# WeiZhang1988/YDORBSLAM

Measured on AMD Instinct MI355X. Metric: ORB extract+match Mkeypoints/sec, higher is better.
Workload: dtype u8

## Files before the change

ydorbslam_amd/csrc/extract_kernels.hip.h:

```cpp
#pragma once
#include <hip/hip_runtime.h>
#include <stdint.h>

#include "quadtree_core.h"
#include "quadtree_flat.h"

#pragma clang fp contract(off)

namespace ydorb {

constexpr int kPad = 19;
constexpr int kBorder = 16;
constexpr int kMaxLevels = 8;
constexpr int kTileMax = 72;
#ifndef QT_THREADS
#define QT_THREADS 512
#endif
constexpr int kQtThreads = QT_THREADS;

struct LevelDev {
  int w, h, pitch;
  int padOff;
  int blurOff, blurPitch;
  int cellBegin, nCells;
  int quota;
  int candOff;
  int kpOff;
  int tabOff;
  int nodeTabOff;
  float scale;
  float size;
};
struct PlanDev {
  int nLevels, nCellsTotal, cellCap, sumQuota;
  int maxX[16];
  unsigned nodeTabFrameStride;
  int blurTileBegin[kMaxLevels + 1];
  int borderBegin[kMaxLevels + 1];
  LevelDev lv[kMaxLevels];
};
#ifndef BLUR_TH
#define BLUR_TH 58
#endif
constexpr int kBlurTW = 64, kBlurTH = BLUR_TH;
struct CellDev {
  short level, x0, y0, x1, y1, pad0;
  int srcOff;
};

__device__ __forceinline__ int reflect101(int i, int n) {
  if (n == 1) return 0;
  while (i < 0 || i >= n) i = i < 0 ? -i : 2 * (n - 1) - i;
  return i;
}

typedef uint32_t __attribute__((aligned(1))) u32_unaligned;
typedef unsigned long long __attribute__((aligned(1))) u64_unaligned;

#ifndef PYR_ROWS
#define PYR_ROWS 8
#endif
constexpr int kPyrRows = PYR_ROWS;
__global__ __launch_bounds__(256) void k_pyr_level0(const uint8_t* __restrict__ img, int stride, size_t frameStride,
                                                    uint8_t* __restrict__ pyr, size_t pyrFrameStride, LevelDev L) {
  const int wx = blockIdx.x * 64 + (threadIdx.x & 63);
  const int yb = (blockIdx.y * 4 + __builtin_amdgcn_readfirstlane(threadIdx.x >> 6)) * kPyrRows;
  const int x0 = wx * 4 - kPad;
  if (x0 + 3 < 0 || x0 >= L.w) return;
  const uint8_t* src = img + (size_t)blockIdx.z * frameStride;
  uint8_t* dst = pyr + (size_t)blockIdx.z * pyrFrameStride + L.padOff + (size_t)kPad * L.pitch + wx * 4;
  const int xa = L.w >= 4 ? min(max(x0, 0), L.w - 4) : 0, sh = 8 * (x0 - xa);
  uint32_t v[kPyrRows];
#pragma unroll
  for (int r = 0; r < kPyrRows; r++) {
    const uint8_t* row = src + (size_t)min(yb + r, L.h - 1) * stride;
    if (L.w >= 4) {
      v[r] = *reinterpret_cast<const u32_unaligned*>(row + xa);
    } else {
      v[r] = 0;
      for (int b = 0; b < L.w; b++) v[r] |= (uint32_t)row[b] << (8 * b);
    }
    v[r] = sh < 0 ? v[r] << (-sh) : v[r] >> sh;
  }
#pragma unroll
  for (int r = 0; r < kPyrRows; r++)
    if (yb + r < L.h) *reinterpret_cast<uint32_t*>(dst + (size_t)(yb + r) * L.pitch) = v[r];
}

__global__ __launch_bounds__(256) void k_pyr_resize(uint8_t* __restrict__ pyr, size_t pyrFrameStride, LevelDev Lp, LevelDev L,
                                                    double scaleX, const short* __restrict__ alpha,
                                                    const int* __restrict__ yofs, const short* __restrict__ beta) {
  const int wx = blockIdx.x * 64 + (threadIdx.x & 63);
  const int yb = (blockIdx.y * 4 + __builtin_amdgcn_readfirstlane(threadIdx.x >> 6)) * kPyrRows;
  const int x0 = wx * 4 - kPad;
  if (x0 + 3 < 0 || x0 >= L.w) return;
  uint8_t* frame = pyr + (size_t)blockIdx.z * pyrFrameStride;
  const uint8_t* S = frame + Lp.padOff + (size_t)kPad * Lp.pitch + kPad;
  uint8_t* dst = frame + L.padOff + (size_t)kPad * L.pitch + wx * 4;
  int sx[4], sx1[4], a0[4], a1[4];
#pragma unroll
  for (int b = 0; b < 4; b++) {
    const int dx = min(max(x0 + b, 0), L.w - 1);
    const float fx = (float)__dsub_rn(__dmul_rn((double)dx + 0.5, scaleX), 0.5);
    sx[b] = min(max((int)floorf(fx), 0), Lp.w - 1);
    a0[b] = alpha[2 * dx]; a1[b] = alpha[2 * dx + 1];
    sx1[b] = min(sx[b] + 1, Lp.w - 1);
  }
  const bool fast = sx[3] - sx[0] <= 6;
  const uint8_t *r0p[kPyrRows], *r1p[kPyrRows];
  int b0[kPyrRows], b1[kPyrRows];
#pragma unroll
  for (int r = 0; r < kPyrRows; r++) {
    const int dy = min(yb + r, L.h - 1);
    const int sy = yofs[dy];
    b0[r] = beta[2 * dy]; b1[r] = beta[2 * dy + 1];
    r0p[r] = S + (size_t)min(max(sy, 0), Lp.h - 1) * Lp.pitch;
    r1p[r] = S + (size_t)min(max(sy + 1, 0), Lp.h - 1) * Lp.pitch;
  }
  uint32_t v[kPyrRows];
  if (fast) {
    typedef unsigned short u16x2 __attribute__((ext_vector_type(2)));
    uint32_t sel[4];
    u16x2 ab[4];
#pragma unroll
    for (int b = 0; b < 4; b++) {
      const uint32_t off = (uint32_t)(sx[b] - sx[0]);
      sel[b] = off | 0x0c000c00u | ((off + 1) << 16);
      ab[b] = u16x2{(unsigned short)a0[b], (unsigned short)a1[b]};
    }
    unsigned long long w0[kPyrRows], w1[kPyrRows];
#pragma unroll
    for (int r = 0; r < kPyrRows; r++) {
      w0[r] = *reinterpret_cast<const u64_unaligned*>(r0p[r] + sx[0]);
      w1[r] = *reinterpret_cast<const u64_unaligned*>(r1p[r] + sx[0]);
    }
#pragma unroll
    for (int r = 0; r < kPyrRows; r++) {
      v[r] = 0;
#pragma unroll
      for (int b = 0; b < 4; b++) {
        const uint32_t p0 = __builtin_amdgcn_perm((uint32_t)(w0[r] >> 32), (uint32_t)w0[r], sel[b]);
        const uint32_t p1 = __builtin_amdgcn_perm((uint32_t)(w1[r] >> 32), (uint32_t)w1[r], sel[b]);
        const int h0 = (int)__builtin_amdgcn_udot2(__builtin_bit_cast(u16x2, p0), ab[b], 0u, false);
        const int h1 = (int)__builtin_amdgcn_udot2(__builtin_bit_cast(u16x2, p1), ab[b], 0u, false);
        const int o = (((b0[r] * (h0 >> 4)) >> 16) + ((b1[r] * (h1 >> 4)) >> 16) + 2) >> 2;
        v[r] |= (uint32_t)(o & 0xFF) << (8 * b);
      }
    }
  } else {
#pragma unroll
    for (int r = 0; r < kPyrRows; r++) {
      v[r] = 0;
#pragma unroll
      for (int b = 0; b < 4; b++) {
        const int h0 = r0p[r][sx[b]] * a0[b] + r0p[r][sx1[b]] * a1[b];
        const int h1 = r1p[r][sx[b]] * a0[b] + r1p[r][sx1[b]] * a1[b];
        const int o = (((b0[r] * (h0 >> 4)) >> 16) + ((b1[r] * (h1 >> 4)) >> 16) + 2) >> 2;
        v[r] |= (uint32_t)(o & 0xFF) << (8 * b);
      }
    }
  }
#pragma unroll
  for (int r = 0; r < kPyrRows; r++)
    if (yb + r < L.h) *reinterpret_cast<uint32_t*>(dst + (size_t)(yb + r) * L.pitch) = v[r];
}

struct PyrPadEntry { uint32_t laneA4, laneB4, selM, selF; };
struct PyrColEntry { uint32_t sel[4]; uint32_t ab[4]; };
constexpr uint32_t kPermIdentity = 0x03020100u;
#ifndef PYR_ROWS_F
#define PYR_ROWS_F 8
#endif
constexpr int kPyrRowsF = PYR_ROWS_F;

__device__ __forceinline__ uint32_t pyr_finish_dword(uint32_t v, const PyrPadEntry& pe) {
  const uint32_t A = (uint32_t)__builtin_amdgcn_ds_bpermute((int)pe.laneA4, (int)v);
  const uint32_t B = (uint32_t)__builtin_amdgcn_ds_bpermute((int)pe.laneB4, (int)v);
  const uint32_t M = __builtin_amdgcn_perm(A, B, pe.selM);
  return __builtin_amdgcn_perm(M, v, pe.selF);
}
__device__ __forceinline__ void pyr_store_rows(uint8_t* dst, int pitch, int y, int h, uint32_t v) {
  if (y >= h) return;
  *reinterpret_cast<uint32_t*>(dst + (ptrdiff_t)y * pitch) = v;
  if (y >= 1 && y <= kPad) *reinterpret_cast<uint32_t*>(dst - (ptrdiff_t)y * pitch) = v;
  if (y >= h - 1 - kPad && y <= h - 2) *reinterpret_cast<uint32_t*>(dst + (ptrdiff_t)(2 * (h - 1) - y) * pitch) = v;
}

__global__ __launch_bounds__(256) void k_pyr_level0_f(const uint8_t* __restrict__ img, int stride, size_t frameStride,
                                                      uint8_t* __restrict__ pyr, size_t pyrFrameStride, LevelDev L,
                                                      const PyrPadEntry* __restrict__ padTab, int shift) {
  const int wx = blockIdx.x * 64 + (threadIdx.x & 63) - shift;
  const int yb = (blockIdx.y * 4 + __builtin_amdgcn_readfirstlane(threadIdx.x >> 6)) * kPyrRowsF;
  const int nd = (L.w + 2 * kPad + 3) >> 2;
  if (wx < 0 || wx >= nd) return;
  const int x0 = wx * 4 - kPad;
  const uint8_t* src = img + (size_t)blockIdx.z * frameStride;
  uint8_t* dst = pyr + (size_t)blockIdx.z * pyrFrameStride + L.padOff + (size_t)kPad * L.pitch + wx * 4;
  typedef uint32_t u32x4 __attribute__((ext_vector_type(4)));
  const u32x4 peRaw = reinterpret_cast<const u32x4*>(padTab)[wx];
  const PyrPadEntry pe{peRaw.x, peRaw.y, peRaw.z, peRaw.w};
  const int xa = min(max(x0, 0), L.w - 4), sh = 8 * (x0 - xa);
  uint32_t v[kPyrRowsF];
#pragma unroll
  for (int r = 0; r < kPyrRowsF; r++) {
    const uint8_t* row = src + (size_t)min(yb + r, L.h - 1) * stride;
    v[r] = *reinterpret_cast<const u32_unaligned*>(row + xa);
  }
  const int shl = min(max(-sh, 0), 31), shr = min(max(sh, 0), 31);
#pragma unroll
  for (int r = 0; r < kPyrRowsF; r++) v[r] = sh < 0 ? v[r] << shl : v[r] >> shr;
  if (__builtin_amdgcn_ballot_w64(pe.selF != kPermIdentity)) {
#pragma unroll
    for (int r = 0; r < kPyrRowsF; r++) v[r] = pyr_finish_dword(v[r], pe);
  }
#pragma unroll
  for (int r = 0; r < kPyrRowsF; r++) pyr_store_rows(dst, L.pitch, yb + r, L.h, v[r]);
}

__global__ __launch_bounds__(256) void k_pyr_resize_f(uint8_t* __restrict__ pyr, size_t pyrFrameStride, LevelDev Lp, LevelDev L,
                                                      double scaleX, const PyrColEntry* __restrict__ colTab,
                                                      const PyrPadEntry* __restrict__ padTab, const int2* __restrict__ rowTab, int shift) {
  const int wx = blockIdx.x * 64 + (threadIdx.x & 63) - shift;
  const int yb = (blockIdx.y * 4 + __builtin_amdgcn_readfirstlane(threadIdx.x >> 6)) * kPyrRowsF;
  const int nd = (L.w + 2 * kPad + 3) >> 2;
  if (wx < 0 || wx >= nd) return;
  uint8_t* frame = pyr + (size_t)blockIdx.z * pyrFrameStride;
  const uint8_t* S = frame + Lp.padOff + (size_t)kPad * Lp.pitch + kPad;
  uint8_t* dst = frame + L.padOff + (size_t)kPad * L.pitch + wx * 4;
  const int dx0 = min(max(wx * 4 - kPad, 0), L.w - 1);
  const float fx = (float)__dsub_rn(__dmul_rn((double)dx0 + 0.5, scaleX), 0.5);
  const int base = min(max((int)floorf(fx), 0), Lp.w - 1);
  const uint8_t* Sb = S + base;
  unsigned long long w0[kPyrRowsF], w1[kPyrRowsF];
  int bw[kPyrRowsF];
#pragma unroll
  for (int r = 0; r < kPyrRowsF; r++) {
    const int2 rt = rowTab[yb + r];
    bw[r] = rt.y;
    w0[r] = *reinterpret_cast<const u64_unaligned*>(Sb + (size_t)min(max(rt.x, 0), Lp.h - 1) * Lp.pitch);
    w1[r] = *reinterpret_cast<const u64_unaligned*>(Sb + (size_t)min(max(rt.x + 1, 0), Lp.h - 1) * Lp.pitch);
  }
  const PyrColEntry ce = colTab[wx];
  typedef uint32_t u32x4 __attribute__((ext_vector_type(4)));
  const u32x4 peRaw = reinterpret_cast<const u32x4*>(padTab)[wx];
  const PyrPadEntry pe{peRaw.x, peRaw.y, peRaw.z, peRaw.w};
  typedef unsigned short u16x2 __attribute__((ext_vector_type(2)));
  uint32_t v[kPyrRowsF];
#pragma unroll
  for (int r = 0; r < kPyrRowsF; r++) {
    const int b0 = bw[r] & 0xffff, b1 = (int)((uint32_t)bw[r] >> 16);
    v[r] = 0;
#pragma unroll
    for (int b = 0; b < 4; b++) {
      const uint32_t p0 = __builtin_amdgcn_perm((uint32_t)(w0[r] >> 32), (uint32_t)w0[r], ce.sel[b]);
      const uint32_t p1 = __builtin_amdgcn_perm((uint32_t)(w1[r] >> 32), (uint32_t)w1[r], ce.sel[b]);
      const int h0 = (int)__builtin_amdgcn_udot2(__builtin_bit_cast(u16x2, p0), __builtin_bit_cast(u16x2, ce.ab[b]), 0u, false);
      const int h1 = (int)__builtin_amdgcn_udot2(__builtin_bit_cast(u16x2, p1), __builtin_bit_cast(u16x2, ce.ab[b]), 0u, false);
      const int o = (((b0 * (h0 >> 4)) >> 16) + ((b1 * (h1 >> 4)) >> 16) + 2) >> 2;
      v[r] |= (uint32_t)(o & 0xFF) << (8 * b);
    }
  }
  if (__builtin_amdgcn_ballot_w64(pe.selF != kPermIdentity)) {
#pragma unroll
    for (int r = 0; r < kPyrRowsF; r++) v[r] = pyr_finish_dword(v[r], pe);
  }
#pragma unroll
  for (int r = 0; r < kPyrRowsF; r++) pyr_store_rows(dst, L.pitch, yb + r, L.h, v[r]);
}

__global__ __launch_bounds__(256) void k_pyr_borders(uint8_t* __restrict__ pyr, size_t pyrFrameStride, PlanDev P) {
  const int f = blockIdx.y;
  int t = blockIdx.x * 256 + threadIdx.x, level = 0;
#pragma unroll
  for (int l = 1; l < kMaxLevels; l++)
    if (l < P.nLevels && (int)(blockIdx.x * 256) >= P.borderBegin[l]) level = l;
  t -= P.borderBegin[level];
  const LevelDev L = P.lv[level];
  const int wd = L.pitch >> 2, rightStart = (kPad + L.w) >> 2;
  constexpr int xdLo = (kPad + 3) / 4;
  const int xdEnd = min(rightStart, wd);
  const int nFast = max(xdEnd - xdLo, 0), nEdge = wd - nFast;
  uint8_t* base = pyr + (size_t)f * pyrFrameStride + L.padOff;
  if (t < 2 * kPad * nFast) {
    const int r = t / nFast, xf = xdLo + t - r * nFast;
    const int yy = r < kPad ? r : L.h + r;
    const int rr = reflect101(yy - kPad, L.h);
    reinterpret_cast<uint32_t*>(base + (size_t)yy * L.pitch)[xf] = reinterpret_cast<const uint32_t*>(base + (size_t)(rr + kPad) * L.pitch)[xf];
    return;
  }
  t -= 2 * kPad * nFast;
  int y, xd;
  if (t < 2 * kPad * nEdge) {
    const int r = t / nEdge, k = t - r * nEdge;
    xd = nFast == 0 ? k : (k < xdLo ? k : xdEnd + k - xdLo);
    y = r < kPad ? r : L.h + r;
  } else {
    const int u = t - 2 * kPad * nEdge, row = u / 12, j = u - row * 12;
    if (row >= L.h) return;
    y = kPad + row;
    xd = j < 6 ? j : rightStart + j - 6;
    if (xd >= wd || (j < 6 && (4 * xd >= kPad || xd >= rightStart))) return;
  }
  uint32_t* dw = reinterpret_cast<uint32_t*>(base + (size_t)y * L.pitch) + xd;
  const int Y = y - kPad, ry = reflect101(Y, L.h);
  const bool rowInside = Y >= 0 && Y < L.h;
  const uint32_t old = rowInside ? *dw : 0u;
  const uint8_t* srow = base + (size_t)(ry + kPad) * L.pitch + kPad;
  uint32_t v = 0;
#pragma unroll
  for (int b = 0; b < 4; b++) {
    const int X = 4 * xd + b - kPad;
    uint32_t px = 0;
    if (X < L.w + kPad) px = (rowInside && X >= 0 && X < L.w) ? (old >> (8 * b)) & 255u : srow[reflect101(X, L.w)];
    v |= px << (8 * b);
  }
  *dw = v;
}

typedef short s16x2 __attribute__((ext_vector_type(2)));
__device__ __forceinline__ s16x2 pk_swap(s16x2 x) { return __builtin_shufflevector(x, x, 1, 0); }
__device__ __forceinline__ s16x2 pk_min(s16x2 a, s16x2 b) { return __builtin_elementwise_min(a, b); }
__device__ __forceinline__ s16x2 pk_max(s16x2 a, s16x2 b) { return __builtin_elementwise_max(a, b); }
__device__ __forceinline__ int fast_arc_best(const s16x2 (&P)[8]) {
  s16x2 pre[8], suf[8];
  pre[0] = P[0];
#pragma unroll
  for (int j = 1; j < 8; j++) pre[j] = pk_min(pre[j - 1], P[j]);
  suf[7] = P[7];
#pragma unroll
  for (int j = 6; j >= 0; j--) suf[j] = pk_min(suf[j + 1], P[j]);
  s16x2 m[8];
#pragma unroll
  for (int j = 0; j < 8; j++) m[j] = pk_min(suf[j], pk_swap(pre[j]));
  const s16x2 r = pk_max(pk_max(pk_max(m[0], m[1]), pk_max(m[2], m[3])), pk_max(pk_max(m[4], m[5]), pk_max(m[6], m[7])));
  return max((int)r.x, (int)r.y);
}

__device__ __forceinline__ int wave_rank(unsigned long long m) {
  return (int)__builtin_amdgcn_mbcnt_hi((unsigned)(m >> 32), __builtin_amdgcn_mbcnt_lo((unsigned)m, 0u));
}

struct FastLds { int tileBytes, scoreBytes, listBytes; };

template <int PITCH>
__global__ __launch_bounds__(256) void k_fast_cells(const uint8_t* __restrict__ pyr, size_t pyrFrameStride, PlanDev P,
                                                    const CellDev* __restrict__ cells, int cellFirst, int cellEnd, int thr, FastLds lds,
                                                    uint32_t* __restrict__ cellCount, uint32_t* __restrict__ cellCand) {
// ... 494 lines not shown
    const uint2 q = *reinterpret_cast<const QT_LDS uint2*>(hist + qf_off(d + 1) + 4 * b);
    const unsigned c0 = q.x & 0xFFFFu, c1 = q.x >> 16, c2 = q.y & 0xFFFFu, c3 = q.y >> 16;
    const unsigned sum = c0 + c1 + c2 + c3;
    hist[qf_off(d) + b] = (uint16_t)sum;
    if (sum >= 2) {
      const unsigned long long nn = (c0 != 0) + (c1 != 0) + (c2 != 0) + (c3 != 0), ll = (c0 == 1) + (c1 == 1) + (c2 == 1) + (c3 == 1);
      const int dd = d + 1;
      if (dd <= 4) { tn0 += nn << (16 * (dd - 1)); tl0 += ll << (16 * (dd - 1)); }
      else { tn1 += nn << (16 * (dd - 5)); tl1 += ll << (16 * (dd - 5)); }
    }
  };
#pragma unroll
  for (int q = 0; q < 4; q++) reduce_level(5, tid + NT * q);
  __syncthreads();
  reduce_level(4, tid);
  __syncthreads();
  if (wv == 0) {
    reduce_level(3, lane);
    __builtin_amdgcn_fence(__ATOMIC_ACQ_REL, "workgroup"); __builtin_amdgcn_wave_barrier();
    if (lane < 16) reduce_level(2, lane);
    __builtin_amdgcn_fence(__ATOMIC_ACQ_REL, "workgroup"); __builtin_amdgcn_wave_barrier();
    if (lane < 4) reduce_level(1, lane);
    __builtin_amdgcn_fence(__ATOMIC_ACQ_REL, "workgroup"); __builtin_amdgcn_wave_barrier();
    if (lane == 0) reduce_level(0, 0);
  }
  tn0 = wave_sum_u64(tn0); tn1 = wave_sum_u64(tn1); tl0 = wave_sum_u64(tl0); tl1 = wave_sum_u64(tl1);
  if (lane == 0) {
    __hip_atomic_fetch_add(&sRed[0], tn0, __ATOMIC_RELAXED, __HIP_MEMORY_SCOPE_WORKGROUP);
    __hip_atomic_fetch_add(&sRed[1], tn1, __ATOMIC_RELAXED, __HIP_MEMORY_SCOPE_WORKGROUP);
    __hip_atomic_fetch_add(&sRed[2], tl0, __ATOMIC_RELAXED, __HIP_MEMORY_SCOPE_WORKGROUP);
    __hip_atomic_fetch_add(&sRed[3], tl1, __ATOMIC_RELAXED, __HIP_MEMORY_SCOPE_WORKGROUP);
  }
  __syncthreads();
  int Pn, K = 0;
  {
    int nodes[D + 1], leaves[D + 1];
    nodes[0] = 1; leaves[0] = 0;
    const unsigned long long a0 = sRed[0], a1 = sRed[1], b0 = sRed[2], b1 = sRed[3];
#pragma unroll
    for (int d = 1; d <= D; d++) {
      nodes[d] = (int)(((d <= 4 ? a0 : a1) >> (16 * ((d - 1) & 3))) & 0xFFFF);
      leaves[d] = (int)(((d <= 4 ? b0 : b1) >> (16 * ((d - 1) & 3))) & 0xFFFF);
    }
    Pn = qt_flat_passes(nodes, leaves, quota, &K, D);
  }
  const bool pairs = Pn < 1;
  if (pairs && n > kQfSmall) { give_up(); return; }
  int nOut = K < quota ? K : quota;
  if (pairs) {
    constexpr int DP = kQtPairDepth, PER = kQfSmall / NT;
    QT_LDS uint32_t* key30 = (QT_LDS uint32_t*)smem;
    QT_LDS unsigned long long* R64 = (QT_LDS unsigned long long*)(smem + 4 * kQfSmall);
    QT_LDS uint8_t* firstOf = (QT_LDS uint8_t*)(smem + 12 * kQfSmall);
    __shared__ int sDiff[kQtPairDepth + 3], sLeaf[kQtPairDepth + 2];
    const int n4 = (n + 3) & ~3;
    uint32_t kk[PER];
    __syncthreads();
    if (tid < DP + 3) sDiff[tid] = 0;
    if (tid < DP + 2) sLeaf[tid] = 0;
#pragma unroll
    for (int t = 0; t < PER; t++) {
      const int i = t * NT + tid;
      kk[t] = i < n ? qt_path_key<kQtPairDepth>(fetch(i), rootX1, rootY1) : 0xFFFFFFFFu;
      if (i < n4) key30[i] = kk[t];
    }
    __syncthreads();
    int sA[PER], eA[PER];
#pragma unroll
    for (int t = 0; t < PER; t++) { sA[t] = 0; eA[t] = 0; }
    for (int q = 0; q < n4; q += 4) {
      const uint4 kq = *reinterpret_cast<const QT_LDS uint4*>(key30 + q);
      const uint32_t ko[4] = {kq.x, kq.y, kq.z, kq.w};
#pragma unroll
      for (int u = 0; u < 4; u++)
#pragma unroll
        for (int t = 0; t < PER; t++) {
          const int i = t * NT + tid;
          const uint32_t x = kk[t] ^ ko[u];
          const int dpt = q + u == i ? 0 : (x ? ((__clz((int)x) - 2) >> 1) + 1 : DP + 1);
          sA[t] = max(sA[t], dpt);
          if (q + u < i) eA[t] = max(eA[t], dpt);
        }
    }
#pragma unroll
    for (int t = 0; t < PER; t++)
      if (t * NT + tid < n) {
        if (eA[t] <= DP) { atomicAdd(&sDiff[eA[t]], 1); atomicAdd(&sDiff[min(sA[t], DP) + 1], -1); }
        if (sA[t] <= DP) atomicAdd(&sLeaf[sA[t]], 1);
      }
    __syncthreads();
    {
      int nodes[DP + 1], leaves[DP + 1], run2 = 0;
#pragma unroll
      for (int d = 0; d <= DP; d++) { run2 += sDiff[d]; nodes[d] = run2; leaves[d] = sLeaf[d]; }
      Pn = qt_flat_passes(nodes, leaves, quota, &K, DP);
    }
    if (Pn < 1) { give_up(); return; }
    nOut = K < quota ? K : quota;
    unsigned long long RR[PER];
#pragma unroll
    for (int t = 0; t < PER; t++) {
      const int i = t * NT + tid, dA = min(Pn, sA[t]);
      RR[t] = ((unsigned long long)(Pn - dA) << (2 * Pn)) | (unsigned long long)((kk[t] >> (2 * (DP - dA))) ^ qt_flat_mask(dA));
      if (i < n4) R64[i] = i < n ? RR[t] : ~0ull;
    }
    __syncthreads();
    bool fst[PER];
#pragma unroll
    for (int t = 0; t < PER; t++) fst[t] = true;
    for (int q = 0; q < n4; q += 2) {
      const ulonglong2 o = *reinterpret_cast<const QT_LDS ulonglong2*>(R64 + q);
      const unsigned long long oo[2] = {o.x, o.y};
#pragma unroll
      for (int u = 0; u < 2; u++)
#pragma unroll
        for (int t = 0; t < PER; t++) fst[t] = fst[t] && !(oo[u] == RR[t] && q + u < t * NT + tid);
    }
#pragma unroll
    for (int t = 0; t < PER; t++) { const int i = t * NT + tid; if (i < n4) firstOf[i] = i < n && fst[t]; }
    __syncthreads();
    int kp[PER], mm[PER];
#pragma unroll
    for (int t = 0; t < PER; t++) { kp[t] = 0; mm[t] = 0; }
    for (int q = 0; q < n4; q += 2) {
      const ulonglong2 o = *reinterpret_cast<const QT_LDS ulonglong2*>(R64 + q);
      const unsigned long long oo[2] = {o.x, o.y};
      const unsigned f2 = *reinterpret_cast<const QT_LDS uint16_t*>(firstOf + q);
#pragma unroll
      for (int u = 0; u < 2; u++)
#pragma unroll
        for (int t = 0; t < PER; t++) {
          kp[t] += (oo[u] < RR[t]) & ((f2 >> (8 * u)) & 1u);
          mm[t] += oo[u] == RR[t];
        }
    }
#pragma unroll
    for (int t = 0; t < PER; t++) {
      const int i = t * NT + tid;
      if (i < n && kp[t] < nOut && mm[t] > 16) nodeBig[kp[t]] = 1;
    }
    static_assert(PER <= ITEMS, "the all-pairs candidates live in the first PER state registers");
#pragma unroll
    for (int t = 0; t < PER; t++) st[t] = (st[t] & 0xFFFF0000u) | (uint32_t)(kp[t] < nOut ? kp[t] : 0x7FFF);
    __syncthreads();
  }

#pragma unroll
  for (int g = 0; g < ITEMS / 4; g++) {
    if (!pairs && 4 * g * NT < n) {
      int key[4], slot[4];
#pragma unroll
      for (int jj = 0; jj < 4; jj++) { key[jj] = (int)(st[4 * g + jj] & 0xFFFu); slot[jj] = qf_off(Pn) + (key[jj] >> (2 * (D - Pn))); }
      for (int d = Pn - 1; d >= 1; d--) {
        const int off = qf_off(d), sh = 2 * (D - d);
#pragma unroll
        for (int jj = 0; jj < 4; jj++) {
          const int sl = off + (key[jj] >> sh);
          if (hist[sl] == 1) slot[jj] = sl;
        }
      }
#pragma unroll
      for (int jj = 0; jj < 4; jj++) st[4 * g + jj] = (st[4 * g + jj] & 0xFFFF0000u) | (uint32_t)slot[jj];
    }
  }
  if (!pairs) {
    const int TQ = ((1 << (2 * Pn)) - 1) / 3;
    const int per = (TQ + NT - 1) / NT;
    constexpr int MAXQ = ((1 << (2 * D)) - 1) / 3 / NT + 1;
    uint2 qv[MAXQ];
    int qslot[MAXQ];
    unsigned flags = 0, cntF = 0;
#pragma unroll
    for (int t = 0; t < MAXQ; t++) {
      qslot[t] = -1; qv[t] = make_uint2(0, 0);
      const int q = tid * per + t;
      if (t < per && q < TQ) {
        int d = Pn, start = 0;
        while (q >= start + (1 << (2 * (d - 1)))) { start += 1 << (2 * (d - 1)); d--; }
        const int pq = q - start;
        const int bq = pq ^ (int)(qt_flat_mask(d) >> 2);
        qslot[t] = qf_off(d) + 4 * bq;
        qv[t] = *reinterpret_cast<const QT_LDS uint2*>(hist + qslot[t]);
        const unsigned c[4] = {qv[t].x & 0xFFFFu, qv[t].x >> 16, qv[t].y & 0xFFFFu, qv[t].y >> 16};
        const unsigned sum = c[0] + c[1] + c[2] + c[3];
#pragma unroll
        for (int e = 0; e < 4; e++) {
          const unsigned cn = c[3 - e];
          const bool fl = sum >= 2 && (d == Pn ? cn >= 1 : cn == 1);
          flags |= (unsigned)fl << (4 * t + e);
          cntF += fl;
        }
      }
    }
    unsigned total;
    unsigned pos = block_scan_excl(cntF, &total);
    if ((int)total != K) { give_up(); return; }
#pragma unroll
    for (int t = 0; t < MAXQ; t++) {
      if (qslot[t] >= 0) {
        const unsigned c[4] = {qv[t].x & 0xFFFFu, qv[t].x >> 16, qv[t].y & 0xFFFFu, qv[t].y >> 16};
        unsigned o[4];
#pragma unroll
        for (int e = 0; e < 4; e++) {
          const unsigned cn = c[3 - e];
          unsigned v = 0x7FFFu;
          if ((flags >> (4 * t + e)) & 1u) {
            if ((int)pos < nOut) {
              v = pos | (cn > 16 ? 0x8000u : 0u);
              if (cn > 16) nodeBig[pos] = 1;
            }
            pos++;
          }
          o[3 - e] = v;
        }
        *reinterpret_cast<QT_LDS uint2*>(hist + qslot[t]) = make_uint2(o[0] | (o[1] << 16), o[2] | (o[3] << 16));
      }
    }
  }
  __syncthreads();

#pragma unroll
  for (int g = 0; g < ITEMS / 4; g++) {
    if (4 * g * NT < n) {
      unsigned pv[4];
#pragma unroll
      for (int jj = 0; jj < 4; jj++) pv[jj] = pairs ? st[4 * g + jj] & 0x7FFFu : hist[st[4 * g + jj] & 0xFFFFu] & 0x7FFFu;
#pragma unroll
      for (int jj = 0; jj < 4; jj++) {
        const int i = (4 * g + jj) * NT + tid;
        const bool ok = i < n && (int)pv[jj] < nOut;
        const unsigned k = ok ? pv[jj] : (unsigned)(quotaMax + 1);
        const uint32_t rs = st[4 * g + jj] & 0xFFFF0000u;
        __hip_atomic_fetch_max(nodeLo + k, ok ? rs | (0xFFFFu - (uint32_t)i) : 0u, __ATOMIC_RELAXED, __HIP_MEMORY_SCOPE_WORKGROUP);
        __hip_atomic_fetch_max(nodeHi + k, ok ? rs | (uint32_t)i : 0u, __ATOMIC_RELAXED, __HIP_MEMORY_SCOPE_WORKGROUP);
        st[4 * g + jj] = rs | (ok ? k : 0xFFFFu);
      }
    }
  }
  __syncthreads();
  for (int k = tid; k < nOut; k += NT) {
    const unsigned iLo = 0xFFFFu - (nodeLo[k] & 0xFFFFu), iHi = nodeHi[k] & 0xFFFFu;
    if (iLo == iHi || !nodeBig[k]) {
      outKp[k] = fetch((int)iLo);
    } else {
      const int s = atomicAdd(&sTieN, 1);
      if (s < kQfMaxTied) { sTieNode[s] = k; nodeBig[k] = (uint8_t)(2 + s); }
    }
  }
  __syncthreads();
  const int nTied = sTieN;
  if (nTied > kQfMaxTied) { give_up(); return; }
  if (nTied > 0) {
    const int slotCap = kQfTieCap / nTied;
    QT_LDS uint32_t* tKey = (QT_LDS uint32_t*)smem;
    QT_LDS uint32_t* tVal = tKey + kQfTieCap;
#pragma unroll
    for (int j = 0; j < ITEMS; j++) {
      if (j * NT < n) {
        const unsigned k = st[j] & 0xFFFFu;
        if (k != 0xFFFFu) {
          const unsigned tb = nodeBig[k];
          if (tb >= 2) {
            const int s = (int)tb - 2, idx = atomicAdd(&sTieCnt[s], 1);
            if (idx < slotCap) { tKey[s * slotCap + idx] = (uint32_t)(j * NT + tid); tVal[s * slotCap + idx] = st[j] >> 16; }
            else sFlag = 1;
          }
        }
      }
    }
    __syncthreads();
    if (sFlag) { give_up(); return; }
    for (int s = 0; s < nTied; s++) {
      const int m = sTieCnt[s];
      constexpr int MAXM = (kQfTieCap + NT - 1) / NT;
      int rk[MAXM];
      uint32_t oi[MAXM], rr[MAXM];
#pragma unroll
      for (int t = 0; t < MAXM; t++) {
        rk[t] = -1; oi[t] = 0; rr[t] = 0;
        const int e = tid + NT * t;
        if (e < m) {
          oi[t] = tKey[s * slotCap + e];
          rr[t] = tVal[s * slotCap + e];
          int r = 0;
          for (int u = 0; u < m; u++) r += tKey[s * slotCap + u] < oi[t];
          rk[t] = r;
        }
      }
      __syncthreads();
#pragma unroll
      for (int t = 0; t < MAXM; t++)
        if (rk[t] >= 0) { tKey[s * slotCap + rk[t]] = (rr[t] << 16) | (uint32_t)rk[t]; tVal[s * slotCap + rk[t]] = oi[t]; }
      __syncthreads();
    }
    if (tid < nTied) {
      const int m = sTieCnt[tid];
      const int best = qt_sort_front(tKey + tid * slotCap, m);
      outKp[sTieNode[tid]] = fetch((int)tVal[tid * slotCap + best]);
    }
  }
  if (tid == 0) { needPass[unit] = 0; lvlCount[unit] = nOut; }
}

__global__ __launch_bounds__(256) void k_blur(const uint8_t* __restrict__ pyr, size_t pyrFrameStride, uint8_t* __restrict__ blur,
                                              size_t blurFrameStride, PlanDev P) {
  constexpr int TW = kBlurTW, TH = kBlurTH, SH = TH + 6, SWW = 18;
  __shared__ uint32_t src[SH * SWW];
  __shared__ __align__(16) uint32_t hb[(SH / 2) * TW];
  int f = blockIdx.y, tileId = blockIdx.x;
  if ((f | 7) < (int)gridDim.y) {
    tileId = (f & 7) * (gridDim.x >> 3) + (blockIdx.x >> 3);
    f = (f & ~7) | (blockIdx.x & 7);
  }
  if (tileId >= P.blurTileBegin[P.nLevels]) return;
  int level = 0;
#pragma unroll
  for (int l = 1; l < kMaxLevels; l++)
    if (l < P.nLevels && tileId >= P.blurTileBegin[l]) level = l;
  tileId -= P.blurTileBegin[level];
  const LevelDev L = P.lv[level];
  const int tilesX = (L.w + TW - 1) / TW;
  const int ty = tileId / tilesX, tx = tileId - ty * tilesX;
  const int x0 = tx * TW, y0 = ty * TH;
  const uint8_t* padded = pyr + (size_t)f * pyrFrameStride + L.padOff;
  {
    const int r0 = threadIdx.x / SWW, wd = threadIdx.x - r0 * SWW;
    const int pcol = x0 + 16 + 4 * wd;
    const bool colOk = pcol < L.pitch;
    if (r0 < 14)
#pragma unroll
      for (int r = r0; r < SH; r += 14) {
        const int prow = min(y0 + r + kPad - 3, L.h + 2 * kPad - 1);
        src[r * SWW + wd] = colOk ? *reinterpret_cast<const uint32_t*>(padded + (size_t)prow * L.pitch + pcol) : 0u;
      }
  }
  __syncthreads();
  for (int task = threadIdx.x; task < (SH / 2) * (TW / 4); task += 256) {
    const int rp = task >> 4, g = task & 15;
    uint32_t o[2][4];
#pragma unroll
    for (int h = 0; h < 2; h++) {
      const int r = 2 * rp + h;
      const uint32_t w0 = src[r * SWW + g], w1 = src[r * SWW + g + 1], w2 = src[r * SWW + g + 2];
#pragma unroll
      for (int k = 0; k < 4; k++) {
        const uint32_t lo4 = k ? __builtin_amdgcn_alignbyte(w1, w0, k) : w0, hi4 = k ? __builtin_amdgcn_alignbyte(w2, w1, k) : w1;
        o[h][k] = __builtin_amdgcn_udot4(hi4, 0x00122230u, __builtin_amdgcn_udot4(lo4, 0x38302212u, 0u, false), false);
      }
    }
    *reinterpret_cast<uint4*>(&hb[rp * TW + g * 4]) =
        make_uint4(o[0][0] | (o[1][0] << 16), o[0][1] | (o[1][1] << 16), o[0][2] | (o[1][2] << 16), o[0][3] | (o[1][3] << 16));
  }
  __syncthreads();
  const int c4 = (threadIdx.x & 15) * 4;
#pragma unroll
  for (int r = threadIdx.x >> 4; r < TH; r += 16) {
    const int gy = y0 + r;
    if (!(gy < L.h && x0 + c4 < L.blurPitch)) continue;
    typedef unsigned short u16x2 __attribute__((ext_vector_type(2)));
    const bool odd = r & 1;
    const u16x2 k0 = odd ? u16x2{0, 18} : u16x2{18, 34}, k1 = odd ? u16x2{34, 48} : u16x2{48, 56};
    const u16x2 k2 = odd ? u16x2{56, 48} : u16x2{48, 34}, k3 = odd ? u16x2{34, 18} : u16x2{18, 0};
    const uint32_t* hp = &hb[(r >> 1) * TW + c4];
    const uint4 p0 = *reinterpret_cast<const uint4*>(hp), p1 = *reinterpret_cast<const uint4*>(hp + TW);
    const uint4 p2 = *reinterpret_cast<const uint4*>(hp + 2 * TW), p3 = *reinterpret_cast<const uint4*>(hp + 3 * TW);
    const uint32_t q0[4] = {p0.x, p0.y, p0.z, p0.w}, q1[4] = {p1.x, p1.y, p1.z, p1.w}, q2[4] = {p2.x, p2.y, p2.z, p2.w}, q3[4] = {p3.x, p3.y, p3.z, p3.w};
    uint32_t acc[4];
#pragma unroll
    for (int k = 0; k < 4; k++) {
      acc[k] = __builtin_amdgcn_udot2(__builtin_bit_cast(u16x2, q0[k]), k0, 32768u, false);
      acc[k] = __builtin_amdgcn_udot2(__builtin_bit_cast(u16x2, q1[k]), k1, acc[k], false);
      acc[k] = __builtin_amdgcn_udot2(__builtin_bit_cast(u16x2, q2[k]), k2, acc[k], false);
      acc[k] = __builtin_amdgcn_udot2(__builtin_bit_cast(u16x2, q3[k]), k3, acc[k], false);
    }
    const uint32_t out = (acc[0] >> 16) | ((acc[1] >> 16) << 8) | ((acc[2] >> 16) << 16) | ((acc[3] >> 16) << 24);
    *reinterpret_cast<uint32_t*>(blur + (size_t)f * blurFrameStride + L.blurOff + (size_t)gy * L.blurPitch + x0 + c4) = out;
  }
}

__device__ __forceinline__ float fast_atan2_deg(float y, float x) {
  const float p1 = 0.9997878412794807f * (float)(180 / 3.14159265358979323846);
  const float p3 = -0.3258083974640975f * (float)(180 / 3.14159265358979323846);
  const float p5 = 0.1555786518463281f * (float)(180 / 3.14159265358979323846);
  const float p7 = -0.04432655554792128f * (float)(180 / 3.14159265358979323846);
  const float eps = (float)2.2204460492503131e-16;
  const float ax = fabsf(x), ay = fabsf(y);
  float a, c, c2;
  if (ax >= ay) {
    c = __fdiv_rn(ay, __fadd_rn(ax, eps));
    c2 = __fmul_rn(c, c);
    a = __fmul_rn(__fadd_rn(__fmul_rn(__fadd_rn(__fmul_rn(__fadd_rn(__fmul_rn(p7, c2), p5), c2), p3), c2), p1), c);
  } else {
    c = __fdiv_rn(ax, __fadd_rn(ay, eps));
    c2 = __fmul_rn(c, c);
    a = __fsub_rn(90.f, __fmul_rn(__fadd_rn(__fmul_rn(__fadd_rn(__fmul_rn(__fadd_rn(__fmul_rn(p7, c2), p5), c2), p3), c2), p1), c));
  }
  if (x < 0) a = __fsub_rn(180.f, a);
  if (y < 0) a = __fsub_rn(360.f, a);
  return a;
}

__device__ __forceinline__ void sincos_det(float xf, float* sinOut, float* cosOut) {
  const double x = (double)xf;
  const double n = rint(__dmul_rn(x, 6.36619772367581382433e-01));
  const double r = __dsub_rn(__dsub_rn(x, __dmul_rn(n, 1.57079632673412561417e+00)), __dmul_rn(n, 6.07710050650619224932e-11));
  const double z = __dmul_rn(r, r);
  double p = __dmul_rn(z, 1.58969099521155010221e-10);
  p = __dadd_rn(p, -2.50507602534068634195e-08); p = __dmul_rn(p, z);
  p = __dadd_rn(p, 2.75573137070700676789e-06);  p = __dmul_rn(p, z);
  p = __dadd_rn(p, -1.98412698298579493134e-04); p = __dmul_rn(p, z);
  p = __dadd_rn(p, 8.33333333332248946124e-03);  p = __dmul_rn(p, z);
  p = __dadd_rn(p, -1.66666666666666324348e-01); p = __dmul_rn(p, z);
  p = __dmul_rn(p, r); p = __dadd_rn(p, r);
  double q = __dmul_rn(z, -1.13596475577881948265e-11);
  q = __dadd_rn(q, 2.08757232129817482790e-09);  q = __dmul_rn(q, z);
  q = __dadd_rn(q, -2.75573143513906633035e-07); q = __dmul_rn(q, z);
  q = __dadd_rn(q, 2.48015872894767294178e-05);  q = __dmul_rn(q, z);
  q = __dadd_rn(q, -1.38888888888741095749e-03); q = __dmul_rn(q, z);
  q = __dadd_rn(q, 4.16666666666666019037e-02);  q = __dmul_rn(q, z);
  q = __dmul_rn(q, z);
  double h = __dmul_rn(z, 0.5);
  h = __dsub_rn(h, q);
  h = __dsub_rn(1.0, h);
  const int quad = ((int)n) & 3;
  const double sv = quad == 0 ? p : quad == 1 ? h : quad == 2 ? -p : -h;
  const double cv = quad == 0 ? h : quad == 1 ? -p : quad == 2 ? -h : p;
  *sinOut = (float)sv;
  *cosOut = (float)cv;
}

__device__ __align__(16) const float kPatternDev[1024] = {
#include "orb_pattern_data.inc"
};

struct YdKeyPointDev { float x, y, size, angle, response; int octave, class_id; };

__global__ __launch_bounds__(256) void k_orient_describe(const uint8_t* __restrict__ pyr, size_t pyrFrameStride,
                                                         const uint8_t* __restrict__ blur, size_t blurFrameStride, PlanDev P,
                                                         const uint32_t* __restrict__ lvlKp, const int* __restrict__ lvlCount,
                                                         YdKeyPointDev* __restrict__ kps, uint8_t* __restrict__ desc, int cap,
                                                         int* __restrict__ nOut, float* __restrict__ lvlAngle) {
  const int lane = threadIdx.x & 63;
  int bx = blockIdx.x, f = blockIdx.y;
  if ((f | 7) < (int)gridDim.y) {
    bx = (f & 7) * (gridDim.x >> 3) + (blockIdx.x >> 3);
    f = (f & ~7) | (blockIdx.x & 7);
  }
  const int slot = bx * 4 + __builtin_amdgcn_readfirstlane(threadIdx.x >> 6);
  if (slot >= P.sumQuota) return;
  float4 pat[4];
#pragma unroll
  for (int t = 0; t < 4; t++) pat[t] = reinterpret_cast<const float4*>(kPatternDev)[t * 64 + lane];
  int level = 0;
#pragma unroll
  for (int l = 1; l < kMaxLevels; l++)
    if (l < P.nLevels && slot >= P.lv[l].kpOff) level = l;
  const uint32_t pk = __builtin_amdgcn_readfirstlane(lvlKp[(size_t)f * P.sumQuota + slot]);
  int before = 0, tot = 0, mine = 0;
#pragma unroll
  for (int l = 0; l < kMaxLevels; l++) {
    const int c = l < P.nLevels ? lvlCount[f * kMaxLevels + l] : 0;
    if (l < level) before += c;
    if (l == level) mine = c;
    tot += c;
  }
  if (slot == 0 && lane == 0) nOut[f] = min(tot, cap);
  const LevelDev L = P.lv[level];
  const int k = slot - L.kpOff;
  if (k >= mine) return;
  const int outIdx = before + k;
  if (outIdx >= cap) return;
  const int kx = qt_x(pk) + kBorder, ky = qt_y(pk) + kBorder;
  const uint8_t* roi = pyr + (size_t)f * pyrFrameStride + L.padOff + (size_t)kPad * L.pitch + kPad;
  const uint8_t* org = roi + (ptrdiff_t)(ky - 15) * L.pitch + (kx - 32);
  const int u = lane - 32;
  unsigned narrow = 0;
#pragma unroll
  for (int v = 1; v <= 15; v++) narrow |= (unsigned)(P.maxX[v] == 0) << v;
  int m10 = 0, m01 = 0;
  if (u >= -15 && u <= 15) m10 = u * org[(unsigned)(15 * L.pitch + lane)];
  if (lane >= 1 && lane <= 15 && ((narrow >> lane) & 1u)) {
    const int pos = org[(unsigned)((15 + lane) * L.pitch + 32)], neg = org[(unsigned)((15 - lane) * L.pitch + 32)];
    m01 = lane * (pos - neg);
  }
#pragma unroll
  for (int v = 1; v <= 15; v++) {
    const int d = P.maxX[v];
    if (d > 0 && u >= -d && u <= d) {
      const int pos = org[(unsigned)((15 + v) * L.pitch + lane)], neg = org[(unsigned)((15 - v) * L.pitch + lane)];
      m01 += v * (pos - neg);
      m10 += u * (pos + neg);
    }
  }
#pragma unroll
  for (int o = 32; o >= 1; o >>= 1) {
    m10 += __shfl_xor(m10, o, 64);
    m01 += __shfl_xor(m01, o, 64);
  }
  const float angle = fast_atan2_deg((float)m01, (float)m10);
  const float rad = __fmul_rn(angle, (float)(3.14159265358979323846 / 180.0));
  float sinB, cosA;
  sincos_det(rad, &sinB, &cosA);
  constexpr int kBias = 24;
  const uint8_t* bl = blur + (size_t)f * blurFrameStride + L.blurOff + (ptrdiff_t)(ky - kBias) * L.blurPitch + (kx - kBias);
  unsigned long long words[4];
#pragma unroll
  for (int t = 0; t < 4; t++) {
    const float4 pt = pat[t];
    const int r0 = __float2int_rn(__fadd_rn(__fmul_rn(pt.x, sinB), __fmul_rn(pt.y, cosA)));
    const int c0 = __float2int_rn(__fsub_rn(__fmul_rn(pt.x, cosA), __fmul_rn(pt.y, sinB)));
    const int r1 = __float2int_rn(__fadd_rn(__fmul_rn(pt.z, sinB), __fmul_rn(pt.w, cosA)));
    const int c1 = __float2int_rn(__fsub_rn(__fmul_rn(pt.z, cosA), __fmul_rn(pt.w, sinB)));
    const int t0 = bl[(unsigned)((r0 + kBias) * L.blurPitch + c0 + kBias)], t1 = bl[(unsigned)((r1 + kBias) * L.blurPitch + c1 + kBias)];
    words[t] = __ballot(t0 < t1);
  }
  if (lane < 4) {
    unsigned long long w = lane == 0 ? words[0] : lane == 1 ? words[1] : lane == 2 ? words[2] : words[3];
    reinterpret_cast<unsigned long long*>(desc + ((size_t)f * cap + outIdx) * 32)[lane] = w;
  }
  if (lane == 0) {
    YdKeyPointDev kp;
    kp.x = (float)kx;
    kp.y = (float)ky;
    if (level) { kp.x = __fmul_rn(kp.x, L.scale); kp.y = __fmul_rn(kp.y, L.scale); }
    kp.size = L.size;
    kp.angle = angle;
    kp.response = (float)qt_r(pk);
    kp.octave = level;
    kp.class_id = -1;
    kps[(size_t)f * cap + outIdx] = kp;
    lvlAngle[(size_t)f * P.sumQuota + slot] = angle;
  }
}


template <int KPW>
__global__ __launch_bounds__(256) void k_orient_describe_n(const uint8_t* __restrict__ pyr, size_t pyrFrameStride,
                                                           const uint8_t* __restrict__ blur, size_t blurFrameStride, PlanDev P,
                                                           const uint32_t* __restrict__ lvlKp, const int* __restrict__ lvlCount,
                                                           YdKeyPointDev* __restrict__ kps, uint8_t* __restrict__ desc, int cap,
                                                           int* __restrict__ nOut, float* __restrict__ lvlAngle) {
  const int lane = threadIdx.x & 63;
  int bx = blockIdx.x, f = blockIdx.y;
  if ((f | 7) < (int)gridDim.y) {
    bx = (f & 7) * (gridDim.x >> 3) + (blockIdx.x >> 3);
    f = (f & ~7) | (blockIdx.x & 7);
  }
  const int slot0 = (bx * 4 + __builtin_amdgcn_readfirstlane(threadIdx.x >> 6)) * KPW;
  if (slot0 >= P.sumQuota) return;
  float4 pat[4];
#pragma unroll
  for (int t = 0; t < 4; t++) pat[t] = reinterpret_cast<const float4*>(kPatternDev)[t * 64 + lane];
  int cnt[kMaxLevels], tot = 0;
#pragma unroll
  for (int l = 0; l < kMaxLevels; l++) { cnt[l] = l < P.nLevels ? lvlCount[f * kMaxLevels + l] : 0; tot += cnt[l]; }
  int level[KPW], outIdx[KPW];
  uint32_t pk[KPW];
  bool valid[KPW];
#pragma unroll
  for (int j = 0; j < KPW; j++) {
    const int slot = min(slot0 + j, P.sumQuota - 1);
    level[j] = 0;
#pragma unroll
    for (int l = 1; l < kMaxLevels; l++)
      if (l < P.nLevels && slot >= P.lv[l].kpOff) level[j] = l;
    pk[j] = __builtin_amdgcn_readfirstlane(lvlKp[(size_t)f * P.sumQuota + slot]);
  }
  if (slot0 == 0 && lane == 0) nOut[f] = min(tot, cap);
  bool any = false;
#pragma unroll
  for (int j = 0; j < KPW; j++) {
    int before = 0, mine = 0;
#pragma unroll
    for (int l = 0; l < kMaxLevels; l++) {
      if (l < level[j]) before += cnt[l];
      if (l == level[j]) mine = cnt[l];
    }
    const int k = slot0 + j - P.lv[level[j]].kpOff;
    outIdx[j] = before + k;
    valid[j] = slot0 + j < P.sumQuota && k < mine && outIdx[j] < cap;
    any = any || valid[j];
  }
  if (!any) return;
  int firstValid = 0;
#pragma unroll
  for (int j = KPW - 1; j >= 0; j--) if (valid[j]) firstValid = j;
#pragma unroll
  for (int j = 0; j < KPW; j++)
    if (!valid[j]) {
#pragma unroll
      for (int i = 0; i < KPW; i++) if (i == firstValid) { pk[j] = pk[i]; level[j] = level[i]; }
    }
  int kx[KPW], ky[KPW], pitch[KPW];
  const uint8_t* org[KPW];
#pragma unroll
  for (int j = 0; j < KPW; j++) {
    const LevelDev& L = P.lv[level[j]];
    kx[j] = qt_x(pk[j]) + kBorder; ky[j] = qt_y(pk[j]) + kBorder;
    pitch[j] = L.pitch;
    const uint8_t* roi = pyr + (size_t)f * pyrFrameStride + L.padOff + (size_t)kPad * L.pitch + kPad;
    org[j] = roi + (ptrdiff_t)(ky[j] - 15) * L.pitch + (kx[j] - 32);
  }
  const int u = lane - 32;
  unsigned narrow = 0;
#pragma unroll
  for (int v = 1; v <= 15; v++) narrow |= (unsigned)(P.maxX[v] == 0) << v;
  int m10[KPW], m01[KPW];
#pragma unroll
  for (int j = 0; j < KPW; j++) {
    m10[j] = 0; m01[j] = 0;
    if (u >= -15 && u <= 15) m10[j] = u * org[j][(unsigned)(15 * pitch[j] + lane)];
    if (lane >= 1 && lane <= 15 && ((narrow >> lane) & 1u)) {
      const int pos = org[j][(unsigned)((15 + lane) * pitch[j] + 32)], neg = org[j][(unsigned)((15 - lane) * pitch[j] + 32)];
      m01[j] = lane * (pos - neg);
    }
  }
#pragma unroll
  for (int v = 1; v <= 15; v++) {
    const int d = P.maxX[v];
    if (d > 0 && u >= -d && u <= d) {
#pragma unroll
      for (int j = 0; j < KPW; j++) {
        const int pos = org[j][(unsigned)((15 + v) * pitch[j] + lane)], neg = org[j][(unsigned)((15 - v) * pitch[j] + lane)];
        m01[j] += v * (pos - neg);
        m10[j] += u * (pos + neg);
      }
    }
  }
#pragma unroll
  for (int o = 32; o >= 1; o >>= 1) {
#pragma unroll
    for (int j = 0; j < KPW; j++) {
      m10[j] += __shfl_xor(m10[j], o, 64);
      m01[j] += __shfl_xor(m01[j], o, 64);
    }
  }
  constexpr int kBias = 24;
  float angle[KPW];
  int tA[KPW][4], tB[KPW][4];
#pragma unroll
  for (int j = 0; j < KPW; j++) {
    const LevelDev& L = P.lv[level[j]];
    angle[j] = fast_atan2_deg((float)m01[j], (float)m10[j]);
    const float rad = __fmul_rn(angle[j], (float)(3.14159265358979323846 / 180.0));
    float sinB, cosA;
    sincos_det(rad, &sinB, &cosA);
    const uint8_t* bl = blur + (size_t)f * blurFrameStride + L.blurOff + (ptrdiff_t)(ky[j] - kBias) * L.blurPitch + (kx[j] - kBias);
#pragma unroll
    for (int t = 0; t < 4; t++) {
      const float4 pt = pat[t];
      const int r0 = __float2int_rn(__fadd_rn(__fmul_rn(pt.x, sinB), __fmul_rn(pt.y, cosA)));
      const int c0 = __float2int_rn(__fsub_rn(__fmul_rn(pt.x, cosA), __fmul_rn(pt.y, sinB)));
      const int r1 = __float2int_rn(__fadd_rn(__fmul_rn(pt.z, sinB), __fmul_rn(pt.w, cosA)));
      const int c1 = __float2int_rn(__fsub_rn(__fmul_rn(pt.z, cosA), __fmul_rn(pt.w, sinB)));
      tA[j][t] = bl[(unsigned)((r0 + kBias) * L.blurPitch + c0 + kBias)];
      tB[j][t] = bl[(unsigned)((r1 + kBias) * L.blurPitch + c1 + kBias)];
    }
  }
#pragma unroll
  for (int j = 0; j < KPW; j++) {
    unsigned long long words[4];
#pragma unroll
    for (int t = 0; t < 4; t++) words[t] = __ballot(tA[j][t] < tB[j][t]);
    if (!valid[j]) continue;
    const LevelDev& L = P.lv[level[j]];
    if (lane < 4) {
      unsigned long long w = lane == 0 ? words[0] : lane == 1 ? words[1] : lane == 2 ? words[2] : words[3];
      reinterpret_cast<unsigned long long*>(desc + ((size_t)f * cap + outIdx[j]) * 32)[lane] = w;
    }
    if (lane == 0) {
      YdKeyPointDev kp;
      kp.x = (float)kx[j];
      kp.y = (float)ky[j];
      if (level[j]) { kp.x = __fmul_rn(kp.x, L.scale); kp.y = __fmul_rn(kp.y, L.scale); }
      kp.size = L.size;
      kp.angle = angle[j];
      kp.response = (float)qt_r(pk[j]);
      kp.octave = level[j];
      kp.class_id = -1;
// ... 8 lines not shown
```

Baseline: 182.9.

## Compute 7x7 Gaussian blur with MFMA f16 banded matrix multiplies

Rewrites the blur kernel so the separable 7-tap Gaussian runs on the matrix cores. Source pixels are converted to f16 and stored column-major in shared memory, and the blur is done with mfma_f32_32x32x16_f16 against precomputed banded coefficient matrices, replacing the udot4/udot2 two-pass integer path. Symmetric rows are pre-added before each multiply. Tile height changes from 58 to 64 rows. The change trades exact integer rounding for f16/f32 arithmetic, which risks small numeric differences. It also adds conversion work and permlane swaps.

```diff
diff --git a/ydorbslam_amd/csrc/extract_kernels.hip.h b/ydorbslam_amd/csrc/extract_kernels.hip.h
--- a/ydorbslam_amd/csrc/extract_kernels.hip.h
+++ b/ydorbslam_amd/csrc/extract_kernels.hip.h
@@ -39,10 +39,7 @@
   int borderBegin[kMaxLevels + 1];
   LevelDev lv[kMaxLevels];
 };
-#ifndef BLUR_TH
-#define BLUR_TH 58
-#endif
-constexpr int kBlurTW = 64, kBlurTH = BLUR_TH;
+constexpr int kBlurTW = 64, kBlurSubH = 64, kBlurSubTiles = 1, kBlurTH = kBlurSubH * kBlurSubTiles;
 struct CellDev {
   short level, x0, y0, x1, y1, pad0;
   int srcOff;
@@ -1143,11 +1140,28 @@
   if (tid == 0) { needPass[unit] = 0; lvlCount[unit] = nOut; }
 }
 
+typedef _Float16 blur_h2 __attribute__((ext_vector_type(2)));
+typedef _Float16 blur_h8 __attribute__((ext_vector_type(8)));
+typedef float blur_f16 __attribute__((ext_vector_type(16)));
+struct alignas(16) BlurBandTab {
+  uint16_t v[3][64][8];
+  constexpr BlurBandTab() : v{} {
+    const uint16_t kv[7] = {0x4C80, 0x5040, 0x5200, 0x5300, 0x5200, 0x5040, 0x4C80};
+    for (int s = 0; s < 3; s++)
+      for (int l = 0; l < 64; l++)
+        for (int e = 0; e < 8; e++) {
+          const int d = 16 * s + 8 * (l >> 5) + e - (l & 31);
+          v[s][l][e] = d >= 0 && d < 7 ? kv[d] : (uint16_t)0;
+        }
+  }
+};
+static __device__ const BlurBandTab kBlurBand{};
+constexpr int kBlurColPitch = 176, kBlurCols = 72;
+
 __global__ __launch_bounds__(256) void k_blur(const uint8_t* __restrict__ pyr, size_t pyrFrameStride, uint8_t* __restrict__ blur,
                                               size_t blurFrameStride, PlanDev P) {
-  constexpr int TW = kBlurTW, TH = kBlurTH, SH = TH + 6, SWW = 18;
-  __shared__ uint32_t src[SH * SWW];
-  __shared__ __align__(16) uint32_t hb[(SH / 2) * TW];
+  constexpr int TW = kBlurTW, TH = kBlurTH, SWW = kBlurCols / 4, CP = kBlurColPitch;
+  __shared__ __align__(16) uint8_t img[kBlurCols * CP];
   int f = blockIdx.y, tileId = blockIdx.x;
   if ((f | 7) < (int)gridDim.y) {
     tileId = (f & 7) * (gridDim.x >> 3) + (blockIdx.x >> 3);
@@ -1164,58 +1178,74 @@
   const int ty = tileId / tilesX, tx = tileId - ty * tilesX;
   const int x0 = tx * TW, y0 = ty * TH;
   const uint8_t* padded = pyr + (size_t)f * pyrFrameStride + L.padOff;
-  {
-    const int r0 = threadIdx.x / SWW, wd = threadIdx.x - r0 * SWW;
-    const int pcol = x0 + 16 + 4 * wd;
-    const bool colOk = pcol < L.pitch;
-    if (r0 < 14)
-#pragma unroll
-      for (int r = r0; r < SH; r += 14) {
-        const int prow = min(y0 + r + kPad - 3, L.h + 2 * kPad - 1);
-        src[r * SWW + wd] = colOk ? *reinterpret_cast<const uint32_t*>(padded + (size_t)prow * L.pitch + pcol) : 0u;
-      }
-  }
-  __syncthreads();
-  for (int task = threadIdx.x; task < (SH / 2) * (TW / 4); task += 256) {
-    const int rp = task >> 4, g = task & 15;
-    uint32_t o[2][4];
-#pragma unroll
-    for (int h = 0; h < 2; h++) {
-      const int r = 2 * rp + h;
-      const uint32_t w0 = src[r * SWW + g], w1 = src[r * SWW + g + 1], w2 = src[r * SWW + g + 2];
-#pragma unroll
-      for (int k = 0; k < 4; k++) {
-        const uint32_t lo4 = k ? __builtin_amdgcn_alignbyte(w1, w0, k) : w0, hi4 = k ? __builtin_amdgcn_alignbyte(w2, w1, k) : w1;
-        o[h][k] = __builtin_amdgcn_udot4(hi4, 0x00122230u, __builtin_amdgcn_udot4(lo4, 0x38302212u, 0u, false), false);
-      }
-    }
-    *reinterpret_cast<uint4*>(&hb[rp * TW + g * 4]) =
-        make_uint4(o[0][0] | (o[1][0] << 16), o[0][1] | (o[1][1] << 16), o[0][2] | (o[1][2] << 16), o[0][3] | (o[1][3] << 16));
-  }
-  __syncthreads();
-  const int c4 = (threadIdx.x & 15) * 4;
-#pragma unroll
-  for (int r = threadIdx.x >> 4; r < TH; r += 16) {
-    const int gy = y0 + r;
-    if (!(gy < L.h && x0 + c4 < L.blurPitch)) continue;
-    typedef unsigned short u16x2 __attribute__((ext_vector_type(2)));
-    const bool odd = r & 1;
-    const u16x2 k0 = odd ? u16x2{0, 18} : u16x2{18, 34}, k1 = odd ? u16x2{34, 48} : u16x2{48, 56};
-    const u16x2 k2 = odd ? u16x2{56, 48} : u16x2{48, 34}, k3 = odd ? u16x2{34, 18} : u16x2{18, 0};
-    const uint32_t* hp = &hb[(r >> 1) * TW + c4];
-    const uint4 p0 = *reinterpret_cast<const uint4*>(hp), p1 = *reinterpret_cast<const uint4*>(hp + TW);
-    const uint4 p2 = *reinterpret_cast<const uint4*>(hp + 2 * TW), p3 = *reinterpret_cast<const uint4*>(hp + 3 * TW);
-    const uint32_t q0[4] = {p0.x, p0.y, p0.z, p0.w}, q1[4] = {p1.x, p1.y, p1.z, p1.w}, q2[4] = {p2.x, p2.y, p2.z, p2.w}, q3[4] = {p3.x, p3.y, p3.z, p3.w};
-    uint32_t acc[4];
-#pragma unroll
-    for (int k = 0; k < 4; k++) {
-      acc[k] = __builtin_amdgcn_udot2(__builtin_bit_cast(u16x2, q0[k]), k0, 32768u, false);
-      acc[k] = __builtin_amdgcn_udot2(__builtin_bit_cast(u16x2, q1[k]), k1, acc[k], false);
-      acc[k] = __builtin_amdgcn_udot2(__builtin_bit_cast(u16x2, q2[k]), k2, acc[k], false);
-      acc[k] = __builtin_amdgcn_udot2(__builtin_bit_cast(u16x2, q3[k]), k3, acc[k], false);
-    }
-    const uint32_t out = (acc[0] >> 16) | ((acc[1] >> 16) << 8) | ((acc[2] >> 16) << 16) | ((acc[3] >> 16) << 24);
-    *reinterpret_cast<uint32_t*>(blur + (size_t)f * blurFrameStride + L.blurOff + (size_t)gy * L.blurPitch + x0 + c4) = out;
+  const int sg = threadIdx.x / SWW, swd = threadIdx.x - sg * SWW;
+  const uint32_t pcol = x0 + 16 + 4 * swd, maxOff = (uint32_t)(L.h + 2 * kPad - 1) * L.pitch + pcol;
+  const bool loads = sg < 9 && (int)pcol < L.pitch;
+  const int wave = __builtin_amdgcn_readfirstlane(threadIdx.x >> 6), wx = wave & 1, wy = wave >> 1;
+  const int lane = threadIdx.x & 63, r = lane & 31, h = lane >> 5;
+  const int tx0 = x0 + 32 * wx;
+  blur_h8 B[4][3];
+#pragma unroll
+  for (int s = 0; s < 3; s++) {
+    const blur_h8 band = __builtin_bit_cast(blur_h8, *reinterpret_cast<const uint4*>(&kBlurBand.v[s][lane][0]));
+    B[0][s] = band * (_Float16)(18.0f / 128);
+    B[1][s] = band * (_Float16)(34.0f / 128);
+    B[2][s] = band * (_Float16)(48.0f / 128);
+    B[3][s] = band * (_Float16)(56.0f / 128);
+  }
+  const uint8_t* ap = &img[(32 * wx + r) * CP + (32 * wy + 8 * h) * 2];
+#pragma unroll 1
+  for (int t = 0; t < kBlurSubTiles; t++) {
+    const int ys = y0 + kBlurSubH * t;
+    if (ys >= L.h) break;
+    if (t) __syncthreads();
+    if (threadIdx.x < 10 * SWW) {
+      uint32_t v[8] = {0u, 0u, 0u, 0u, 0u, 0u, 0u, 0u};
+      if (loads) {
+        const uint32_t off = (uint32_t)(ys + 8 * sg + kPad - 3) * L.pitch + pcol;
+#pragma unroll
+        for (int q = 0; q < 8; q++) v[q] = *reinterpret_cast<const uint32_t*>(padded + min(off + (uint32_t)(q * L.pitch), maxOff));
+      }
+      const blur_h2 up = {(_Float16)32768.0f, (_Float16)32768.0f};
+#pragma unroll
+      for (int c = 0; c < 4; c++) {
+        const uint32_t sel = 0x0c040c00u + (uint32_t)c * 0x00010001u;
+        uint32_t o[4];
+#pragma unroll
+        for (int q = 0; q < 4; q++)
+          o[q] = __builtin_bit_cast(uint32_t, __builtin_bit_cast(blur_h2, __builtin_amdgcn_perm(v[2 * q + 1], v[2 * q], sel)) * up);
+        *reinterpret_cast<uint4*>(&img[(4 * swd + c) * CP + 16 * sg]) = make_uint4(o[0], o[1], o[2], o[3]);
+      }
+    }
+    __syncthreads();
+    const int gy = ys + 32 * wy + r;
+    const bool active = ys + 32 * wy < L.h && tx0 < L.blurPitch;
+    uint32_t d[4] = {0u, 0u, 0u, 0u};
+    if (active) {
+      blur_f16 acc;
+#pragma unroll
+      for (int g = 0; g < 16; g++) acc[g] = 0.5f;
+#pragma unroll
+      for (int i = 0; i < 4; i++)
+#pragma unroll
+        for (int s = 0; s < 3; s++) {
+          blur_h8 a = *reinterpret_cast<const blur_h8*>(ap + i * CP + 32 * s);
+          if (i < 3) a += *reinterpret_cast<const blur_h8*>(ap + (6 - i) * CP + 32 * s);
+          acc = __builtin_amdgcn_mfma_f32_32x32x16_f16(a, B[i][s], acc, 0, 0, 0);
+        }
+#pragma unroll
+      for (int q = 0; q < 4; q++) {
+        const uint32_t b0 = (uint32_t)acc[4 * q], b1 = (uint32_t)acc[4 * q + 1], b2 = (uint32_t)acc[4 * q + 2], b3 = (uint32_t)acc[4 * q + 3];
+        d[q] = b0 | (b1 << 8) | (b2 << 16) | (b3 << 24);
+      }
+      {
+        const auto s0 = __builtin_amdgcn_permlane32_swap(d[0], d[2], false, false);
+        const auto s1 = __builtin_amdgcn_permlane32_swap(d[1], d[3], false, false);
+        d[0] = s0[0]; d[1] = s0[1]; d[2] = s1[0]; d[3] = s1[1];
+      }
+    }
+    if (active && gy < L.h)
+      *reinterpret_cast<uint4*>(blur + (size_t)f * blurFrameStride + L.blurOff + (uint32_t)(gy * L.blurPitch + tx0 + 16 * h)) = make_uint4(d[0], d[1], d[2], d[3]);
   }
 }
 
```

New measurement: 182.9 (median of 2 runs). No clear change (+0.0%).
